# Kyaw-Thiha/animal-vision

Measured on AMD Instinct MI355X. Metric: megapixels/sec per-frame pipeline, higher is better.
Workload: dtype f16

## Files before the change

### animal-vision_amd/csrc/mst_fused.hip

```cpp
#include <hip/hip_fp16.h>

#include <cstdio>
#include <cstdlib>
#include <cstring>

#include "avx_internal.h"
#include "mst_common.h"
#include "mst_tile_order.h"

namespace {

typedef float float4_t __attribute__((ext_vector_type(4)));
#ifndef AVX_FFN32_GM2
#define AVX_FFN32_GM2 1
#endif
constexpr int kFT = 512;
constexpr int TS = 16;
constexpr int HS = TS + 2;
#ifndef AVX_FFN_TH
#define AVX_FFN_TH 16
#endif
constexpr int kFfnTH = AVX_FFN_TH;
static_assert(kFfnTH == 14 || kFfnTH == 16, "FeedForward tile rows");
constexpr int kFfnNGRP = (HS * (kFfnTH + 2) + 31) / 32;

__device__ __forceinline__ float16_t mfma16(half8_t a, half8_t b, float16_t c) { return __builtin_amdgcn_mfma_f32_32x32x16_f16(a, b, c, 0, 0, 0); }

struct Tile { int x0, y0; long b; };
template <class Walk>
__device__ __forceinline__ Tile tile_at(const Walk& wk, int side_x, int side_y) { return Tile{wk.xi * side_x, wk.yi * side_y, (long)wk.b}; }
int mst_tile_order() {
    const char* e = getenv("AVX_MST_TILE_ORDER");
    return e && !strcmp(e, "raster") ? AVX_TILE_ORDER_RASTER : AVX_TILE_ORDER_XCD;
}

typedef _Float16 half16_t __attribute__((ext_vector_type(16)));
template <bool DWS>
__device__ __forceinline__ float4_t dw_unit(const half8_t (&a)[3], const uint4 (&bq)[3]) {
    float4_t acc = {0.f, 0.f, 0.f, 0.f};
    if constexpr (DWS) {
        const half8_t b0 = __builtin_bit_cast(half8_t, bq[0]), b1 = __builtin_bit_cast(half8_t, bq[1]);
        acc = __builtin_amdgcn_mfma_f32_16x16x32_f16(a[1], __builtin_bit_cast(half8_t, bq[2]), acc, 0, 0, 0);
        acc = __builtin_amdgcn_smfmac_f32_16x16x64_f16(a[0], __builtin_shufflevector(b0, b1, 0, 1, 2, 3, 4, 5, 6, 7, 8, 9, 10, 11, 12, 13, 14, 15), acc,
                                                       (int)__builtin_bit_cast(uint4, a[2]).x, 0, 0);
    } else {
#pragma unroll
        for (int i = 0; i < 3; ++i) acc = __builtin_amdgcn_mfma_f32_16x16x32_f16(a[i], __builtin_bit_cast(half8_t, bq[i]), acc, 0, 0, 0);
    }
    return acc;
}
template <bool DWS>
__device__ __forceinline__ half8_t dw_frag(const uint4* p, int i) {
    if (DWS && i == 2) return __builtin_bit_cast(half8_t, uint4{*reinterpret_cast<const unsigned*>(p), 0u, 0u, 0u});
    return __builtin_bit_cast(half8_t, *p);
}
template <bool MARCH> struct FfnWalk { typedef TileWalk type; };
template <> struct FfnWalk<true> { typedef ColumnWalk type; };
template <int C, int HPASS, int MINW, bool DWM, bool STAMP = false, int NW = 8, bool DWS = false, bool MARCH = false>
__global__ __launch_bounds__(64 * NW, MINW) void k_mst_ffn_fused(const __half* __restrict__ x , const float* __restrict__ gamma, const float* __restrict__ beta,
                                                          float eps, const uint4* __restrict__ w1pack , const __half* __restrict__ taps ,
                                                          const uint4* __restrict__ w2pack , __half* __restrict__ out , int B,
                                                          int H, int W, const uint4* __restrict__ dwpack , unsigned long long* __restrict__ stamps , int order ) {
    constexpr int FTH = MARCH ? 14 : kFfnTH, HSY = FTH + 2, ROW0 = MARCH ? 2 : 0, NHALO = HS * (HSY - ROW0), NGRP = (NHALO + 31) / 32;
    constexpr int HID = 4 * C, NPASS = HID / HPASS, KS1 = C / 16, KS2 = HPASS / 16, NT = C / 32, YPITCH = C * 2 + 16, LNV = C / 16;
    constexpr int HPITCH = HPASS * 2 + 16, RPITCH = (HS * HPITCH + 255) / 256 * 256 , NCT = HPASS / 32;
    static_assert(C == 32 || C == 64 || C == 128, "31-, 62- or 124-channel blocks (stored 32 / 64 / 128 wide)");
    constexpr int NTHR = 64 * NW, NGW = (NGRP + NW - 1) / NW;
    constexpr int NTW = NT / (NW / 8), NOCTW = HPASS / (8 * NW);
    static_assert((NW == 8 || NW == 16) && NT % (NW / 8) == 0 && (!DWM || HPASS % (8 * NW) == 0) && (DWM || NW == 8) && (DWM || !DWS) && (DWM || !MARCH), "wave split");
    constexpr bool PREFETCH = C <= 64;
    extern __shared__ __align__(16) unsigned char smem[];
    unsigned char* yt = smem;
    unsigned char* ht = yt + (size_t)NGRP * 32 * YPITCH;
    __half* tapl = reinterpret_cast<__half*>(ht + (size_t)HSY * RPITCH);
    float* gl = reinterpret_cast<float*>(tapl + (DWM ? 0 : 9 * HID));
    constexpr bool W2LDS = NW == 16;
    uint4* w2l = reinterpret_cast<uint4*>(gl + 2 * C);
    constexpr int NPRIME = 2 * HS, CARRY = NPRIME * HPITCH;
    unsigned char* carry = reinterpret_cast<unsigned char*>(w2l + (W2LDS ? NT * KS2 * 64 : 0));
    const int tid = threadIdx.x, lane = tid & 63, wave = tid >> 6, p = lane & 31, h = lane >> 5;
    unsigned long long seg[8] = {0, 0, 0, 0, 0, 0, 0, 0}, tlast = 0;
    auto stamp = [&](int k) {
        if constexpr (STAMP) {
            const unsigned long long now = __builtin_readcyclecounter();
            seg[k] += now - tlast;
            tlast = now;
        }
    };
    if constexpr (STAMP) tlast = __builtin_readcyclecounter();
    if constexpr (!DWM)
        for (int i = tid; i < 9 * HID; i += NTHR) tapl[i] = taps[i];
    for (int i = tid; i < C; i += NTHR) { gl[i] = gamma[i]; gl[C + i] = beta[i]; }
    const int tx = (W + TS - 1) / TS, ty = (H + FTH - 1) / FTH;
    const float cnt = (float)(NT * 31);

    uint4 raw[NGW][LNV];
    unsigned f_rel[NGW];
#pragma unroll
    for (int gi = 0; gi < NGW; ++gi) {
        const int q = 32 * (wave + NW * gi) + p, qq = q < NHALO ? q : NHALO - 1;
        f_rel[gi] = (unsigned)(((qq / HS) * W + qq % HS) * C + h * (C / 2)) * 2u;
    }
    auto fetch = [&](const Tile& t) {
        if (t.y0 + ROW0 >= 1 && t.y0 + HSY - 1 <= H && t.x0 >= 1 && t.x0 + HS - 1 <= W) {
            const char* origin = reinterpret_cast<const char*>(x + ((t.b * H + t.y0 - 1 + ROW0) * (size_t)W + t.x0 - 1) * C);
#pragma unroll
            for (int gi = 0; gi < NGW; ++gi) {
                if (wave + NW * gi >= NGRP) break;
                unsigned o = f_rel[gi];
                asm volatile("" : "+v"(o));
                const uint4* src = reinterpret_cast<const uint4*>(origin + o);
#pragma unroll
                for (int v = 0; v < LNV; ++v) raw[gi][v] = src[v];
            }
            return;
        }
#pragma unroll
        for (int gi = 0; gi < NGW; ++gi) {
            const int g = wave + NW * gi;
            if (g >= NGRP) break;
            const int q = 32 * g + p, qq = q < NHALO ? q : NHALO - 1;
            int yy = t.y0 - 1 + ROW0 + qq / HS, xx = t.x0 - 1 + qq % HS;
            yy = yy < 0 ? 0 : (yy >= H ? H - 1 : yy);
            xx = xx < 0 ? 0 : (xx >= W ? W - 1 : xx);
            const uint4* src = reinterpret_cast<const uint4*>(x + ((t.b * H + yy) * (size_t)W + xx) * C + h * (C / 2));
#pragma unroll
            for (int v = 0; v < LNV; ++v) raw[gi][v] = src[v];
        }
    };
    constexpr int NGPRIME = (NPRIME + 31) / 32;
    auto fetch_prime = [&](const Tile& t) {
        if (wave >= NGPRIME) return;
        int td = tid;
        asm volatile("" : "+v"(td));
        const int q = 32 * (td >> 6) + (td & 31), qq = q < NPRIME ? q : NPRIME - 1, hl = (td >> 5) & 1;
        int yy = t.y0 - 1 + qq / HS, xx = t.x0 - 1 + qq % HS;
        yy = yy < 0 ? 0 : (yy >= H ? H - 1 : yy);
        xx = xx < 0 ? 0 : (xx >= W ? W - 1 : xx);
        const uint4* src = reinterpret_cast<const uint4*>(x + ((t.b * H + yy) * (size_t)W + xx) * C + hl * (C / 2));
#pragma unroll
        for (int v = 0; v < LNV; ++v) raw[0][v] = src[v];
    };
    auto layernorm = [&](int ngrp) {
        if constexpr (DWM) {
#pragma unroll
            for (int gi = 0; gi < NGW; ++gi) {
                const int g = wave + NW * gi;
                if (g >= ngrp) break;
                typedef _Float16 half2v __attribute__((ext_vector_type(2)));
                constexpr unsigned kOnes = 0x3c003c00u;
                auto is_pad = [&](int i) { return ((h * (C / 2) + i) & 31) == 31; };
                auto word = [&](int i) { const uint4 u = raw[gi][i / 8]; const int k = (i / 2) & 3; return k == 0 ? u.x : k == 1 ? u.y : k == 2 ? u.z : u.w; };
                float s1 = 0.f;
#pragma unroll
                for (int i = 0; i < 8 * LNV; i += 2) s1 = __builtin_amdgcn_fdot2(__builtin_bit_cast(half2v, word(i)), __builtin_bit_cast(half2v, kOnes), s1, false);
                const float mean = (s1 + __shfl_xor(s1, 32)) / cnt, nmean = -mean;
                float d[8 * LNV], s2 = 0.f;
#pragma unroll
                for (int i = 0; i < 8 * LNV; ++i) {
                    const float t = (i & 1) ? fma_mix_hi_c(word(i), kOnes, nmean) : fma_mix_lo_c(word(i), kOnes, nmean);
                    d[i] = is_pad(i) ? 0.f : t;
                    s2 = __builtin_fmaf(d[i], d[i], s2);
                }
                const float rstd = rsqrtf((s2 + __shfl_xor(s2, 32)) / cnt + eps);
                int pl = p;
                if constexpr (MARCH) asm volatile("" : "+v"(pl));
                unsigned char* dst = yt + (size_t)(32 * g + pl) * YPITCH + h * C;
#pragma unroll
                for (int v = 0; v < LNV; ++v) {
                    unsigned o[4];
#pragma unroll
                    for (int j = 0; j < 8; j += 2) {
                        const int i = 8 * v + j;
                        const float2_t y2 = float2_t{d[i], d[i + 1]} * float2_t{rstd, rstd};
                        const float bq = (h * (C / 2) + i + 1) == 31 ? 1.0f : y2.y;
                        o[j / 2] = pack_f16(y2.x, bq);
                    }
                    *reinterpret_cast<uint4*>(dst + 16 * v) = uint4{o[0], o[1], o[2], o[3]};
                }
            }
            return;
        }
#pragma unroll
        for (int gi = 0; gi < NGW; ++gi) {
            const int g = wave + NW * gi;
            if (g >= NGRP) break;
            constexpr unsigned kOnes = 0x3c003c00u;
            auto is_pad = [&](int i) { return ((h * (C / 2) + i) & 31) == 31; };
            auto word = [&](int i) { const uint4 u = raw[gi][i / 8]; const int k = (i / 2) & 3; return k == 0 ? u.x : k == 1 ? u.y : k == 2 ? u.z : u.w; };
            float s1 = 0.f;
#pragma unroll
            for (int i = 0; i < 8 * LNV; ++i) {
                const float t = (i & 1) ? fma_mix_hi_c(word(i), kOnes, s1) : fma_mix_lo_c(word(i), kOnes, s1);
                s1 = is_pad(i) ? s1 : t;
            }
            const float mean = (s1 + __shfl_xor(s1, 32)) / cnt, nmean = -mean;
            float d[8 * LNV], s2 = 0.f;
#pragma unroll
            for (int i = 0; i < 8 * LNV; ++i) {
                const float t = (i & 1) ? fma_mix_hi_c(word(i), kOnes, nmean) : fma_mix_lo_c(word(i), kOnes, nmean);
                d[i] = is_pad(i) ? 0.f : t;
                s2 = __builtin_fmaf(d[i], d[i], s2);
            }
            const float rstd = rsqrtf((s2 + __shfl_xor(s2, 32)) / cnt + eps);
            unsigned char* dst = yt + (size_t)(32 * g + p) * YPITCH + h * C;
#pragma unroll
            for (int v = 0; v < LNV; ++v) {
                unsigned o[4];
#pragma unroll
                for (int j = 0; j < 8; j += 2) {
                    const int i = 8 * v + j, c = h * (C / 2) + i;
                    const float a = is_pad(i) ? 0.f : __builtin_fmaf(d[i] * rstd, gl[c], gl[C + c]);
                    const float bq = is_pad(i + 1) ? 0.f : __builtin_fmaf(d[i + 1] * rstd, gl[c + 1], gl[C + c + 1]);
                    o[j / 2] = pack_f16(a, bq);
                }
                *reinterpret_cast<uint4*>(dst + 16 * v) = uint4{o[0], o[1], o[2], o[3]};
            }
        }
    };

    const int n0 = (wave / 8) * NTW, w8 = wave % 8;
    half8_t w2f[W2LDS ? 1 : NTW * KS2];
    auto load_w2 = [&](int pass) {
#pragma unroll
        for (int n = 0; n < NTW; ++n)
#pragma unroll
            for (int s = 0; s < KS2; ++s) w2f[n * KS2 + s] = __builtin_bit_cast(half8_t, w2pack[((size_t)(n0 + n) * (HID / 16) + pass * KS2 + s) * 64 + lane]);
    };
    if constexpr (NPASS == 1 && !W2LDS) load_w2(0);
    half8_t w1f[KS1];
    auto load_w1 = [&](int pass) {
#pragma unroll
        for (int s = 0; s < KS1; ++s) w1f[s] = __builtin_bit_cast(half8_t, w1pack[((size_t)(pass * NCT + wave % NCT) * KS1 + s) * 64 + lane]);
    };
    constexpr bool W1AHEAD = DWM && C == 64 && NPASS > 1 && NW == 8;
    static_assert(!(MARCH && W1AHEAD), "the marching form loads W1 at the top of phase 1 (priming replaces the fragments)");
    if constexpr (W1AHEAD) load_w1(0);
    constexpr int NITEM = (NGRP + NW / NCT - 1) / (NW / NCT);
    int p1_g[NITEM], p1_dst[NITEM], p1_dy[NITEM], p1_dx[NITEM];
#pragma unroll
    for (int j = 0; j < NITEM; ++j) {
        const int g = wave / NCT + j * (NW / NCT), q = 32 * g + p, qc = q < NHALO ? q : 0;
        p1_g[j] = g < NGRP ? g : -1;
        p1_dst[j] = (g < NGRP && q < NHALO) ? (ROW0 + qc / HS) * RPITCH + (qc % HS) * HPITCH + 32 * h : -1;
        p1_dy[j] = ROW0 + qc / HS - 1; p1_dx[j] = qc % HS - 1;
    }
    auto p1_item = [&](int g, unsigned char* base, int off, bool masked, int yy, int xx) {
        float16_t d;
#pragma unroll
        for (int v = 0; v < 16; ++v) d[v] = 0.f;
        const unsigned char* ysrc = yt + (size_t)(32 * g + p) * YPITCH + 16 * h;
#pragma unroll
        for (int s = 0; s < KS1; ++s) d = mfma16(w1f[s], __builtin_bit_cast(half8_t, *reinterpret_cast<const uint4*>(ysrc + 32 * s)), d);
        if (off >= 0) {
            unsigned char* dst = base + off;
            uint32_t keep = 0xffffffffu;
            if (masked) keep = (yy >= 0 && yy < H && xx >= 0 && xx < W) ? 0xffffffffu : 0u;
            constexpr int GP1 = (C == 64 && NW == 8) ? 4 : (C == 32 ? 2 : 1);
            unsigned pk[8];
#pragma unroll
            for (int v0 = 0; v0 < 8; v0 += GP1) {
                float2_t gq[GP1];
#pragma unroll
                for (int v = 0; v < GP1; ++v) gq[v] = float2_t{d[2 * (v0 + v)], d[2 * (v0 + v) + 1]};
                if constexpr (DWM) gelu_mx<GP1>(gq); else gelu_multi<GP1>(gq);
#pragma unroll
                for (int v = 0; v < GP1; ++v) pk[v0 + v] = pack_f16(gq[v].x, gq[v].y);
            }
            uint4 u0 = uint4{pk[0], pk[1], pk[2], pk[3]}, u1 = uint4{pk[4], pk[5], pk[6], pk[7]};
            if (masked) { u0.x &= keep; u0.y &= keep; u0.z &= keep; u0.w &= keep; u1.x &= keep; u1.y &= keep; u1.z &= keep; u1.w &= keep; }
            reinterpret_cast<uint4*>(dst)[0] = u0;
            reinterpret_cast<uint4*>(dst)[1] = u1;
        }
    };
    auto prime = [&](const Tile& t) {
        fetch_prime(t);
        layernorm(NGPRIME);
        __syncthreads();
        const int g = wave / NCT;
        int td = tid;
        asm volatile("" : "+v"(td));
        const int wl = td >> 6, q = 32 * (wl / NCT) + (td & 31), qc = q < NPRIME ? q : 0, yy = t.y0 - 1 + qc / HS, xx = t.x0 - 1 + qc % HS;
        const int off = q < NPRIME ? qc * HPITCH + 32 * ((td >> 5) & 1) + 64 * (wl % NCT) : -1;
        if (g < NGPRIME) {
#pragma unroll 1
            for (int pass = 0; pass < NPASS; ++pass) {
                load_w1(pass);
                p1_item(g, carry + (size_t)pass * CARRY, off, true, yy, xx);
            }
        }
        __syncthreads();
    };
    typename FfnWalk<MARCH>::type ahead;
    if constexpr (MARCH) ahead.init(blockIdx.x, gridDim.x, B, ty, tx);
    else ahead.init(blockIdx.x, gridDim.x, B, ty, tx, order);
    if (!ahead.live) return;
    Tile t = tile_at(ahead, TS, FTH);
    ahead.advance();
    if constexpr (MARCH) prime(t);
    fetch(t);
    __syncthreads();
    layernorm(NGRP);
    for (;;) {
        const bool halo_inside = t.y0 + ROW0 >= 1 && t.y0 + HSY - 1 <= H && t.x0 >= 1 && t.x0 + HS - 1 <= W;
        float16_t D[NTW];
#pragma unroll
        for (int n = 0; n < NTW; ++n)
#pragma unroll
            for (int v = 0; v < 16; ++v) D[n][v] = 0.f;
#pragma unroll 1
        for (int pass = 0; pass < NPASS; ++pass) {
            stamp(pass == 0 ? 7 : 5);
            __syncthreads();
            stamp(0);
            if constexpr (W2LDS)
                for (int i = tid; i < NT * KS2 * 64; i += NTHR) w2l[i] = w2pack[((size_t)(i / (KS2 * 64)) * (HID / 16) + pass * KS2 + (i / 64) % KS2) * 64 + (i & 63)];
            half8_t af[DWM ? NOCTW : 1][3];
            if constexpr (DWM) {
#pragma unroll
                for (int o2 = 0; o2 < NOCTW; ++o2)
#pragma unroll
                    for (int i = 0; i < 3; ++i) af[o2][i] = dw_frag<DWS>(dwpack + ((size_t)(pass * (HPASS / 8) + NW * o2 + wave) * 3 + i) * 64 + lane, i);
            }
            {
                const int ct = wave % NCT;
                if constexpr (!W1AHEAD) load_w1(pass);
                if constexpr (MARCH) {
                    constexpr int NV = NPRIME * (HPASS / 8);
                    static_assert(NV <= NTHR, "one 16-byte piece per thread");
                    int i = tid;
                    asm volatile("" : "+v"(i));
                    if (i < NV) {
                        const int px = i / (HPASS / 8), o = i % (HPASS / 8);
                        *reinterpret_cast<uint4*>(ht + (size_t)(px / HS) * RPITCH + (size_t)(px % HS) * HPITCH + 16 * o) =
                            *reinterpret_cast<const uint4*>(carry + (size_t)pass * CARRY + (size_t)px * HPITCH + 16 * o);
                    }
                }
#pragma unroll
                for (int j = 0; j < NITEM; ++j) {
                    if (p1_g[j] < 0) continue;
                    p1_item(p1_g[j], ht + 64 * ct, p1_dst[j], !halo_inside, t.y0 + p1_dy[j], t.x0 + p1_dx[j]);
                }
            }
            stamp(1);
            __syncthreads();
            stamp(2);
            bool ahead_fetch = ahead.live;
            if constexpr (MARCH) ahead_fetch = ahead_fetch && !ahead.seg;
            if (PREFETCH && pass == NPASS - 1 && ahead_fetch) fetch(tile_at(ahead, TS, FTH));
            if constexpr (NPASS > 1 && !W2LDS) load_w2(pass);
            if constexpr (DWM) {
                constexpr int NOCT = NOCTW;
                const int n16 = lane & 15, q = lane >> 4;
                unsigned char* rbase = ht + (size_t)q * RPITCH + (size_t)n16 * HPITCH + 16 * wave;
                unsigned char* wbase = ht + (size_t)(q >> 1) * RPITCH + (size_t)n16 * HPITCH + 16 * wave + 8 * (q & 1);
                constexpr int NU = NOCT * (FTH / 2);
                uint4 bq[3];
                auto rd = [&](int u) {
                    const int o2 = u / (FTH / 2), pr = u % (FTH / 2);
#pragma unroll
                    for (int i = 0; i < 3; ++i) bq[i] = *reinterpret_cast<const uint4*>(rbase + (size_t)(2 * pr) * RPITCH + (size_t)i * HPITCH + 16 * NW * o2);
                };
                auto finish = [&](int u, float4_t a) {
                    const int o2 = u / (FTH / 2), pr = u % (FTH / 2);
                    float2_t gp[2] = {float2_t{a[0], a[1]}, float2_t{a[2], a[3]}};
                    if constexpr (C == 64 || (C == 32 && AVX_FFN32_GM2)) gelu_mx<2>(gp);
                    else { float2_t g0[1] = {gp[0]}, g1[1] = {gp[1]}; gelu_mx<1>(g0); gelu_mx<1>(g1); gp[0] = g0[0]; gp[1] = g1[0]; }
                    *reinterpret_cast<uint2*>(wbase + (size_t)(2 * pr) * RPITCH + 16 * NW * o2) = uint2{pack_f16(gp[0].x, gp[0].y), pack_f16(gp[1].x, gp[1].y)};
                };
#ifndef AVX_FFN_PIPE_ALL
#define AVX_FFN_PIPE_ALL 0
#endif
#ifndef AVX_FFN_MARCH_PIPE32
#define AVX_FFN_MARCH_PIPE32 1
#endif
                constexpr bool PIPE = C == 64 || AVX_FFN_PIPE_ALL || (MARCH && C == 32 && AVX_FFN_MARCH_PIPE32);
                if constexpr (PIPE) {
                    rd(0);
                    float4_t prev = {0.f, 0.f, 0.f, 0.f};
#pragma unroll
                    for (int u = 0; u < NU; ++u) {
                        const int o2 = u / (FTH / 2);
                        const float4_t acc = dw_unit<DWS>(af[o2], bq);
                        if (u + 1 < NU) rd(u + 1);
                        __builtin_amdgcn_sched_barrier(0);
                        if (u > 0) finish(u - 1, prev);
                        __builtin_amdgcn_sched_barrier(0);
                        prev = acc;
                    }
                    finish(NU - 1, prev);
                } else {
#pragma unroll
                    for (int u = 0; u < NU; ++u) {
                        const int o2 = u / (FTH / 2);
                        rd(u);
                        const float4_t acc = dw_unit<DWS>(af[o2], bq);
                        finish(u, acc);
                    }
                }
                stamp(3);
                __syncthreads();
                stamp(4);
                if constexpr (W1AHEAD) load_w1(pass + 1 < NPASS ? pass + 1 : 0);
                const int r = 2 * w8 + (p >> 4), c = p & 15;
                const unsigned char* zb = ht + (size_t)r * RPITCH + (size_t)c * HPITCH + 16 * h;
                constexpr int NVC = NPRIME * (HPASS / 8);
                constexpr bool SPREAD = MARCH && !W2LDS;
                uint4 cv = uint4{0u, 0u, 0u, 0u};
                int ci = tid;
                if constexpr (SPREAD) {
                    asm volatile("" : "+v"(ci));
                    if (ci < NVC) cv = *reinterpret_cast<const uint4*>(ht + (size_t)(FTH + (ci / (HPASS / 8)) / HS) * RPITCH + (size_t)((ci / (HPASS / 8)) % HS) * HPITCH + 16 * (ci % (HPASS / 8)));
                }
                if (SPREAD || 2 * w8 < FTH) {
#pragma unroll
                for (int s = 0; s < KS2; ++s) {
                    const half8_t bf = __builtin_bit_cast(half8_t, *reinterpret_cast<const uint4*>(zb + 32 * s));
#pragma unroll
                    for (int n = 0; n < NTW; ++n) {
                        if constexpr (W2LDS) D[n] = mfma16(__builtin_bit_cast(half8_t, w2l[((n0 + n) * KS2 + s) * 64 + lane]), bf, D[n]);
                        else D[n] = mfma16(w2f[n * KS2 + s], bf, D[n]);
                    }
                }
                }
                if constexpr (SPREAD) {
                    if (ci < NVC) *reinterpret_cast<uint4*>(carry + (size_t)pass * CARRY + (size_t)(ci / (HPASS / 8)) * HPITCH + 16 * (ci % (HPASS / 8))) = cv;
                } else if constexpr (MARCH) {
                    if (2 * w8 >= FTH)
                        for (int i = (wave / 8) * 64 + lane; i < NVC; i += 64 * (NW / 8)) {
                            const int px = i / (HPASS / 8), o = i % (HPASS / 8);
                            *reinterpret_cast<uint4*>(carry + (size_t)pass * CARRY + (size_t)px * HPITCH + 16 * o) =
                                *reinterpret_cast<const uint4*>(ht + (size_t)(FTH + px / HS) * RPITCH + (size_t)(px % HS) * HPITCH + 16 * o);
                        }
                }
            } else
            if (2 * wave < FTH) {
                const int r = 2 * wave + (p >> 4), c = p & 15;
                const unsigned char* hbase = ht + (size_t)r * RPITCH + (size_t)c * HPITCH + 16 * h;
                const unsigned char* tbase = reinterpret_cast<const unsigned char*>(tapl) + (size_t)(pass * HPASS + 8 * h) * 2;
#pragma unroll
                for (int s = 0; s < KS2; ++s) {
                    float acc[8];
#pragma unroll
                    for (int j = 0; j < 8; ++j) acc[j] = 0.f;
#pragma unroll
                    for (int tap = 0; tap < 9; ++tap) {
                        const uint4 hv = *reinterpret_cast<const uint4*>(hbase + (size_t)(tap / 3) * RPITCH + (size_t)(tap % 3) * HPITCH + 32 * s);
                        const uint4 wv = *reinterpret_cast<const uint4*>(tbase + (size_t)tap * HID * 2 + 32 * s);
                        fma_mix_lo(acc[0], hv.x, wv.x); fma_mix_hi(acc[1], hv.x, wv.x);
                        fma_mix_lo(acc[2], hv.y, wv.y); fma_mix_hi(acc[3], hv.y, wv.y);
                        fma_mix_lo(acc[4], hv.z, wv.z); fma_mix_hi(acc[5], hv.z, wv.z);
                        fma_mix_lo(acc[6], hv.w, wv.w); fma_mix_hi(acc[7], hv.w, wv.w);
                    }
                    half8_t bf;
#pragma unroll
                    for (int j = 0; j < 8; j += 2) {
                        const float2_t gv = gelu_fast2(float2_t{acc[j], acc[j + 1]});
                        bf[j] = (_Float16)gv.x;
                        bf[j + 1] = (_Float16)gv.y;
                    }
#pragma unroll
                    for (int n = 0; n < NT; ++n)
                        D[n] = mfma16(w2f[n * KS2 + s], bf, D[n]);
                }
            }
        }
        stamp(5);
        {
            const int yo = t.y0 + 2 * w8 + (p >> 4), xo = t.x0 + (p & 15);
            if (2 * w8 < FTH && yo < H && xo < W) {
                const size_t off = ((t.b * H + yo) * (size_t)W + xo) * C + 16 * h + 32 * n0;
#pragma unroll
                for (int n = 0; n < NTW; ++n) {
                    const uint4 xa = reinterpret_cast<const uint4*>(x + off + 32 * n)[0], xb = reinterpret_cast<const uint4*>(x + off + 32 * n)[1];
                    const unsigned xw[8] = {xa.x, xa.y, xa.z, xa.w, xb.x, xb.y, xb.z, xb.w};
                    unsigned ow[8];
#pragma unroll
                    for (int j = 0; j < 8; ++j) {
                        float s0 = D[n][2 * j], s1 = D[n][2 * j + 1];
                        fma_mix_lo(s0, xw[j], 0x3c003c00u); fma_mix_hi(s1, xw[j], 0x3c003c00u);
                        ow[j] = pack_f16(s0, s1);
                    }
                    reinterpret_cast<uint4*>(out + off + 32 * n)[0] = uint4{ow[0], ow[1], ow[2], ow[3]};
                    reinterpret_cast<uint4*>(out + off + 32 * n)[1] = uint4{ow[4], ow[5], ow[6], ow[7]};
                }
            }
        }
        stamp(6);
        if (!ahead.live) break;
        t = tile_at(ahead, TS, FTH);
        bool fetch_now = !PREFETCH;
        if constexpr (MARCH) {
            if (ahead.seg) { prime(t); fetch_now = true; }
        }
        ahead.advance();
        if (fetch_now) fetch(t);
        layernorm(NGRP);
    }
    if constexpr (STAMP) {
        if (lane == 0 && stamps)
#pragma unroll
            for (int k = 0; k < 8; ++k) stamps[((size_t)blockIdx.x * NW + wave) * 8 + k] = seg[k];
    }
}


constexpr int VS = TS + 4, MS = TS + 2;

template <int C, int MINW>
__global__ __launch_bounds__(kFT, MINW) void k_mst_attn_tail(const __half* __restrict__ v , const __half* __restrict__ x ,
                                                             const uint4* __restrict__ mpack , const __half* __restrict__ taps1 ,
                                                             const __half* __restrict__ taps2 , const float* __restrict__ bias ,
                                                             __half* __restrict__ out, int B, int H, int W, const uint4* __restrict__ wvpack ) {
    constexpr int NO = C / 8, NS = C / 16, NT = C / 32, PP = C * 2 + 16;
    constexpr int VRP = (VS * PP + 255) / 256 * 256, MRP = VRP;
    constexpr int NFILL = (VS * VS * NO + kFT - 1) / kFT;
    extern __shared__ __align__(16) unsigned char smem[];
    unsigned char* vt = smem;
    unsigned char* mt = vt + (size_t)VS * VRP;
    const bool fromx = wvpack != nullptr;
    __half* t2l = reinterpret_cast<__half*>(mt + (size_t)VS * VRP);
    __half* t1l = t2l + 9 * C;
    float* bl = reinterpret_cast<float*>(t1l + 9 * C);
    const int tid = threadIdx.x, lane = tid & 63, wave = tid >> 6, p = lane & 31, h = lane >> 5;
// ... 1387 lines not shown
}

extern "C" int avx_mst_ffn_fused(avx_ctx* ctx, const void* x, const float* gamma, const float* beta, float eps, const void* w1pack, const void* taps_9xhid,
                                 const void* w2pack, void* out, int B, int H, int W, int C, void* stream) {
    if (!ctx) return AVX_ERR_INVALID;
    AVX_REQUIRE(ctx, taps_9xhid, "avx_mst_ffn_fused: NULL pointer");
    return ffn_fused_launch(ctx, x, gamma, beta, eps, w1pack, taps_9xhid, nullptr, w2pack, out, B, H, W, C, stream);
}

extern "C" int avx_mst_ffn_fused_mx(avx_ctx* ctx, const void* x, const float* gamma, const float* beta, float eps, const void* w1pack, const void* dwpack,
                                    const void* w2pack, void* out, int B, int H, int W, int C, void* stream) {
    if (!ctx) return AVX_ERR_INVALID;
    AVX_REQUIRE(ctx, dwpack && (((uintptr_t)dwpack) & 15u) == 0, "avx_mst_ffn_fused_mx: dwpack NULL or not 16-byte aligned");
    return ffn_fused_launch(ctx, x, gamma, beta, eps, w1pack, nullptr, dwpack, w2pack, out, B, H, W, C, stream);
}

extern "C" int avx_mst_ffn_fused_sp(avx_ctx* ctx, const void* x, const float* gamma, const float* beta, float eps, const void* w1pack, const void* dwpack,
                                    const void* w2pack, void* out, int B, int H, int W, int C, void* stream) {
    if (!ctx) return AVX_ERR_INVALID;
    AVX_REQUIRE(ctx, dwpack && (((uintptr_t)dwpack) & 15u) == 0, "avx_mst_ffn_fused_sp: dwpack NULL or not 16-byte aligned");
    return ffn_fused_launch(ctx, x, gamma, beta, eps, w1pack, nullptr, dwpack, w2pack, out, B, H, W, C, stream, true);
}

extern "C" int avx_mst_ffn_fused_mx_col(avx_ctx* ctx, const void* x, const float* gamma, const float* beta, float eps, const void* w1pack, const void* dwpack,
                                        const void* w2pack, void* out, int B, int H, int W, int C, int max_workgroups, void* stream) {
    if (!ctx) return AVX_ERR_INVALID;
    AVX_REQUIRE(ctx, dwpack && (((uintptr_t)dwpack) & 15u) == 0, "avx_mst_ffn_fused_mx_col: dwpack NULL or not 16-byte aligned");
    AVX_REQUIRE(ctx, (C == 32 || C == 64) && max_workgroups >= 0, "avx_mst_ffn_fused_mx_col: C=%d (32 or 64), max_workgroups=%d (>= 0)", C, max_workgroups);
    return ffn_fused_launch(ctx, x, gamma, beta, eps, w1pack, nullptr, dwpack, w2pack, out, B, H, W, C, stream, false, true, max_workgroups);
}
extern "C" int avx_mst_ffn_fused_sp_col(avx_ctx* ctx, const void* x, const float* gamma, const float* beta, float eps, const void* w1pack, const void* dwpack,
                                        const void* w2pack, void* out, int B, int H, int W, int C, int max_workgroups, void* stream) {
    if (!ctx) return AVX_ERR_INVALID;
    AVX_REQUIRE(ctx, dwpack && (((uintptr_t)dwpack) & 15u) == 0, "avx_mst_ffn_fused_sp_col: dwpack NULL or not 16-byte aligned");
    AVX_REQUIRE(ctx, (C == 32 || C == 64) && max_workgroups >= 0, "avx_mst_ffn_fused_sp_col: C=%d (32 or 64), max_workgroups=%d (>= 0)", C, max_workgroups);
    return ffn_fused_launch(ctx, x, gamma, beta, eps, w1pack, nullptr, dwpack, w2pack, out, B, H, W, C, stream, true, true, max_workgroups);
}

static int ffn_fused_launch(avx_ctx* ctx, const void* x, const float* gamma, const float* beta, float eps, const void* w1pack, const void* taps_9xhid, const void* dwpack,
                            const void* w2pack, void* out, int B, int H, int W, int C, void* stream, bool sparse, bool march, int max_workgroups) {
    AVX_REQUIRE(ctx, x && gamma && beta && w1pack && w2pack && out && B > 0 && H > 0 && W > 0, "avx_mst_ffn_fused: NULL pointer or empty tensor");
    AVX_REQUIRE(ctx, C == 32 || C == 64 || C == 128, "avx_mst_ffn_fused: C=%d (32, 64 or 128: 31-channel groups stored 32 wide)", C);
    AVX_REQUIRE(ctx, ((((uintptr_t)x | (uintptr_t)w1pack | (uintptr_t)w2pack | (uintptr_t)out | (uintptr_t)taps_9xhid)) & 15u) == 0,
                "avx_mst_ffn_fused: pointers must be 16-byte aligned");
    AVX_REQUIRE(ctx, x != out, "avx_mst_ffn_fused: neighbouring tiles read each other's halo: the output cannot be the input");
    AVX_HIP(ctx, hipSetDevice(ctx->device));
    hipStream_t s = avx_pick_stream(ctx, stream);
    const int fth = march ? 14 : kFfnTH;
    const long total = (long)B * ((H + fth - 1) / fth) * ((W + TS - 1) / TS);
    const char* hp = getenv("AVX_MST_FFN_HPASS");
    const bool small = C == 32 && (march || !(hp && atoi(hp) == 128));
    const int hpass = (small || C == 128) ? 64 : 128, hpitch = hpass * 2 + 16, rpitch = (HS * hpitch + 255) / 256 * 256;
    const long cap = (long)ctx->num_cus * (small ? 2 : 1);
    const bool nw16 = C == 64 && dwpack && (march || !(getenv("AVX_MST_FFN_NW") && atoi(getenv("AVX_MST_FFN_NW")) == 8));
    const size_t lds = (size_t)(march ? 8 : kFfnNGRP) * 32 * (C * 2 + 16) + (size_t)(fth + 2) * rpitch + (dwpack ? 0 : (size_t)9 * 4 * C * 2) + sizeof(float) * 2 * C +
                       (nw16 ? (size_t)(C / 32) * (hpass / 16) * 1024 : 0) + (march ? (size_t)(4 * C / hpass) * 2 * HS * hpitch : 0);
    AVX_REQUIRE(ctx, total <= 0x7fffffffl, "avx_mst_ffn_fused: 2^31 tiles or more");
    AVX_REQUIRE(ctx, !march || (dwpack && (C == 32 || C == 64)), "avx_mst_ffn_fused: the marching form is built for the matrix-pipe kernels at C = 32 and 64");
    long nwg = total < cap ? total : cap;
    if (max_workgroups > 0 && max_workgroups < nwg) nwg = max_workgroups;
    const dim3 grid((unsigned)nwg);
    const int order = mst_tile_order();
#define AVX_FFN1M(CV, HP, MW, DW, NWV, SP, MR)                                                                                                   \
    {                                                                                                                                            \
        auto k = k_mst_ffn_fused<CV, HP, MW, DW, false, NWV, SP, MR>;                                                                            \
        AVX_HIP(ctx, hipFuncSetAttribute((const void*)k, hipFuncAttributeMaxDynamicSharedMemorySize, (int)lds));                                 \
        hipLaunchKernelGGL(k, grid, dim3(64 * NWV), lds, s, (const __half*)x, gamma, beta, eps, (const uint4*)w1pack, (const __half*)taps_9xhid, \
                           (const uint4*)w2pack, (__half*)out, B, H, W, (const uint4*)dwpack, (unsigned long long*)nullptr, order);              \
    }
#define AVX_FFN1S(CV, HP, MW, DW, NWV, SP) AVX_FFN1M(CV, HP, MW, DW, NWV, SP, false)
#define AVX_FFN1(CV, HP, MW, DW, NWV) AVX_FFN1S(CV, HP, MW, DW, NWV, false)
#define AVX_FFN(CV, HP, MW) { if (dwpack && sparse) AVX_FFN1S(CV, HP, MW, true, 8, true) else if (dwpack) AVX_FFN1(CV, HP, MW, true, 8) else AVX_FFN1(CV, HP, MW, false, 8) }
    if (dwpack && getenv("AVX_FFN_STAMPS") && ((C == 32 && small) || C == 64 || C == 128)) {
        unsigned long long* d_st = nullptr;
        const int nwv = nw16 ? 16 : 8;
        const size_t n = (size_t)grid.x * nwv * 8;
        AVX_HIP(ctx, hipMalloc((void**)&d_st, n * sizeof(unsigned long long)));
#define AVX_FFN_ST2(CV, HP, MW, NWV, SP, MR)                                                                                                     \
    {                                                                                                                                            \
        auto k = k_mst_ffn_fused<CV, HP, MW, true, true, NWV, SP, MR>;                                                                           \
        AVX_HIP(ctx, hipFuncSetAttribute((const void*)k, hipFuncAttributeMaxDynamicSharedMemorySize, (int)lds));                                 \
        hipLaunchKernelGGL(k, grid, dim3(64 * NWV), lds, s, (const __half*)x, gamma, beta, eps, (const uint4*)w1pack, (const __half*)taps_9xhid, \
                           (const uint4*)w2pack, (__half*)out, B, H, W, (const uint4*)dwpack, d_st, order);                                      \
    }
#define AVX_FFN_ST1(CV, HP, MW, NWV, SP) AVX_FFN_ST2(CV, HP, MW, NWV, SP, false)
#define AVX_FFN_ST(CV, HP, MW, NWV) { if (sparse) AVX_FFN_ST1(CV, HP, MW, NWV, true) else AVX_FFN_ST1(CV, HP, MW, NWV, false) }
#define AVX_FFN_STM(CV, HP, MW, NWV) { if (sparse) AVX_FFN_ST2(CV, HP, MW, NWV, true, true) else AVX_FFN_ST2(CV, HP, MW, NWV, false, true) }
        if (march && C == 32) AVX_FFN_STM(32, 64, 4, 8) else if (march) AVX_FFN_STM(64, 128, 1, 16)
        else if (C == 32) AVX_FFN_ST(32, 64, 4, 8) else if (nw16) AVX_FFN_ST(64, 128, 1, 16) else if (C == 64) AVX_FFN_ST(64, 128, 2, 8) else AVX_FFN_ST(128, 64, 2, 8)
#undef AVX_FFN_STM
#undef AVX_FFN_ST
#undef AVX_FFN_ST1
#undef AVX_FFN_ST2
        AVX_HIP(ctx, hipStreamSynchronize(s));
        unsigned long long* h_st = (unsigned long long*)malloc(n * sizeof(unsigned long long));
        AVX_HIP(ctx, hipMemcpy(h_st, d_st, n * sizeof(unsigned long long), hipMemcpyDeviceToHost));
        double tot[8] = {0}, w0[8] = {0}, w7[8] = {0};
        for (size_t i = 0; i < n; ++i) { tot[i & 7] += (double)h_st[i]; if (((i >> 3) % nwv) == 0) w0[i & 7] += (double)h_st[i]; if (((i >> 3) % nwv) == (size_t)nwv - 1) w7[i & 7] += (double)h_st[i]; }
        double all = 0;
        for (int k2 = 0; k2 < 8; ++k2) all += tot[k2];
        fprintf(stderr, "[ffn stamps C=%d%s] %u blocks x %d waves, mean cycles per wave %.0f; share per segment (all waves | first wave | last wave): ", C, march ? " march" : "", grid.x, nwv, all / (grid.x * (double)nwv));
        const char* nm[8] = {"bar1", "phase1", "bar2", "phase2a", "bar3", "phase2b", "epilogue", "ln+fetch"};
        for (int k2 = 0; k2 < 8; ++k2) fprintf(stderr, "%s %.1f%% | %.1f%% | %.1f%%  ", nm[k2], 100 * tot[k2] / all, 100 * w0[k2] * nwv / all, 100 * w7[k2] * nwv / all);
        fprintf(stderr, "\n");
        free(h_st);
        (void)hipFree(d_st);
    } else if (march && C == 32 && sparse) AVX_FFN1M(32, 64, 4, true, 8, true, true)
    else if (march && C == 32) AVX_FFN1M(32, 64, 4, true, 8, false, true)
    else if (march && sparse) AVX_FFN1M(64, 128, 1, true, 16, true, true)
    else if (march) AVX_FFN1M(64, 128, 1, true, 16, false, true)
    else if (C == 32 && small) AVX_FFN(32, 64, 4) else if (C == 32) AVX_FFN(32, 128, 2)
    else if (nw16 && sparse) AVX_FFN1S(64, 128, 1, true, 16, true)
    else if (nw16) AVX_FFN1(64, 128, 1, true, 16)
    else if (C == 64) AVX_FFN(64, 128, 2) else AVX_FFN(128, 64, 2)
#undef AVX_FFN
#undef AVX_FFN1
#undef AVX_FFN1S
#undef AVX_FFN1M
    AVX_HIP(ctx, hipGetLastError());
    return AVX_OK;
}

extern "C" int avx_mst_attn_tail(avx_ctx* ctx, const void* v, const void* x, const void* mpack16, const void* taps1_9xc, const void* taps2_9xc, const float* bias,
                                 void* out, int B, int H, int W, int C, void* stream) {
    if (!ctx) return AVX_ERR_INVALID;
    AVX_REQUIRE(ctx, v && x && mpack16 && taps1_9xc && taps2_9xc && out && B > 0 && H > 0 && W > 0, "avx_mst_attn_tail: NULL pointer or empty tensor");
    AVX_REQUIRE(ctx, C == 32 || C == 64, "avx_mst_attn_tail: C=%d (32 or 64)", C);
    AVX_REQUIRE(ctx, ((((uintptr_t)v | (uintptr_t)x | (uintptr_t)mpack16 | (uintptr_t)out | (uintptr_t)taps1_9xc | (uintptr_t)taps2_9xc)) & 15u) == 0,
                "avx_mst_attn_tail: pointers must be 16-byte aligned");
    AVX_REQUIRE(ctx, v != out, "avx_mst_attn_tail: tiles read their neighbours' rows of v: the output cannot be v (it may be x)");
    AVX_HIP(ctx, hipSetDevice(ctx->device));
    hipStream_t s = avx_pick_stream(ctx, stream);
    if (C == 32) return launch_attn_tail<32, 4>(ctx, v, x, mpack16, taps1_9xc, taps2_9xc, bias, out, B, H, W, s, nullptr);
    return launch_attn_tail<64, 2>(ctx, v, x, mpack16, taps1_9xc, taps2_9xc, bias, out, B, H, W, s, nullptr);
}

extern "C" int avx_mst_attn_tail_x(avx_ctx* ctx, const void* x, const void* wvpack16, const void* mpack16, const void* taps1_9xc, const void* taps2_9xc,
                                   const float* bias, void* out, int B, int H, int W, int C, void* stream) {
    if (!ctx) return AVX_ERR_INVALID;
    AVX_REQUIRE(ctx, x && wvpack16 && mpack16 && taps1_9xc && taps2_9xc && out && B > 0 && H > 0 && W > 0, "avx_mst_attn_tail_x: NULL pointer or empty tensor");
    AVX_REQUIRE(ctx, C == 32 || C == 64, "avx_mst_attn_tail_x: C=%d (32 or 64)", C);
    AVX_REQUIRE(ctx, ((((uintptr_t)x | (uintptr_t)wvpack16 | (uintptr_t)mpack16 | (uintptr_t)out | (uintptr_t)taps1_9xc | (uintptr_t)taps2_9xc)) & 15u) == 0,
                "avx_mst_attn_tail_x: pointers must be 16-byte aligned");
    AVX_REQUIRE(ctx, x != out, "avx_mst_attn_tail_x: tiles read their neighbours' rows of x: the output cannot be x");
    AVX_HIP(ctx, hipSetDevice(ctx->device));
    hipStream_t s = avx_pick_stream(ctx, stream);
    if (C == 32) return launch_attn_tail<32, 4>(ctx, x, x, mpack16, taps1_9xc, taps2_9xc, bias, out, B, H, W, s, wvpack16);
    return launch_attn_tail<64, 2>(ctx, x, x, mpack16, taps1_9xc, taps2_9xc, bias, out, B, H, W, s, wvpack16);
}

template <bool DWS>
static int attn_tail_mx_launch(avx_ctx* ctx, const void* x, const void* wvpack16, const void* mpack_mx, const void* dw1pack, const void* dw2pack, const float* bias, void* out,
                               int B, int H, int W, int C, void* stream) {
    AVX_REQUIRE(ctx, x && wvpack16 && mpack_mx && dw1pack && dw2pack && out && B > 0 && H > 0 && W > 0, "avx_mst_attn_tail_mx: NULL pointer or empty tensor");
    AVX_REQUIRE(ctx, C == 32 || C == 64 || C == 128, "avx_mst_attn_tail_mx: C=%d (32, 64 or 128)", C);
    AVX_REQUIRE(ctx, ((((uintptr_t)x | (uintptr_t)wvpack16 | (uintptr_t)mpack_mx | (uintptr_t)out | (uintptr_t)dw1pack | (uintptr_t)dw2pack)) & 15u) == 0,
                "avx_mst_attn_tail_mx: pointers must be 16-byte aligned");
    AVX_REQUIRE(ctx, x != out, "avx_mst_attn_tail_mx: tiles read their neighbours' rows of x: the output cannot be x");
    AVX_HIP(ctx, hipSetDevice(ctx->device));
    hipStream_t s = avx_pick_stream(ctx, stream);
    if (C == 32) return launch_attn_tail_mx<32, 16, 4, 8, DWS>(ctx, x, wvpack16, mpack_mx, dw1pack, dw2pack, bias, out, B, H, W, s);
    if (C == 128) return launch_attn_tail_mx<128, 8, 2, 8, DWS>(ctx, x, wvpack16, mpack_mx, dw1pack, dw2pack, bias, out, B, H, W, s);
    if (getenv("AVX_MST_TAIL_NW") && atoi(getenv("AVX_MST_TAIL_NW")) == 16) return launch_attn_tail_mx<64, 16, 1, 16, DWS>(ctx, x, wvpack16, mpack_mx, dw1pack, dw2pack, bias, out, B, H, W, s);
    return launch_attn_tail_mx<64, 16, 2, 8, DWS>(ctx, x, wvpack16, mpack_mx, dw1pack, dw2pack, bias, out, B, H, W, s);
// ... 256 lines not shown
```

Baseline: 456.5.

## Run C=128 FeedForward with 16 waves, splitting depthwise row pairs across two waves

```diff
diff --git a/animal-vision_amd/csrc/mst_fused.hip b/animal-vision_amd/csrc/mst_fused.hip
--- a/animal-vision_amd/csrc/mst_fused.hip
+++ b/animal-vision_amd/csrc/mst_fused.hip
@@ -3,6 +3,7 @@
 #include <cstdio>
 #include <cstdlib>
 #include <cstring>
+#include <type_traits>
 
 #include "avx_internal.h"
 #include "mst_common.h"
@@ -66,16 +67,31 @@
     constexpr int HPITCH = HPASS * 2 + 16, RPITCH = (HS * HPITCH + 255) / 256 * 256 , NCT = HPASS / 32;
     static_assert(C == 32 || C == 64 || C == 128, "31-, 62- or 124-channel blocks (stored 32 / 64 / 128 wide)");
     constexpr int NTHR = 64 * NW, NGW = (NGRP + NW - 1) / NW;
-    constexpr int NTW = NT / (NW / 8), NOCTW = HPASS / (8 * NW);
-    static_assert((NW == 8 || NW == 16) && NT % (NW / 8) == 0 && (!DWM || HPASS % (8 * NW) == 0) && (DWM || NW == 8) && (DWM || !DWS) && (DWM || !MARCH), "wave split");
-    constexpr bool PREFETCH = C <= 64;
+    constexpr bool SPLIT = DWM && 2 * HPASS == 8 * NW;
+    constexpr int NTW = NT / (NW / 8), NOCTW = SPLIT ? 1 : HPASS / (8 * NW);
+    static_assert((NW == 8 || NW == 16) && NT % (NW / 8) == 0 && (!DWM || SPLIT || HPASS % (8 * NW) == 0) && (DWM || NW == 8) && (DWM || !DWS) && (DWM || !MARCH), "wave split");
+    static_assert(!SPLIT || (!MARCH && FTH == 16 && NW == 16), "two waves per octet: 8 row pairs, 4 each");
+#ifndef AVX_FFN128_PREFETCH
+#define AVX_FFN128_PREFETCH 0
+#endif
+#ifndef AVX_FFN128_PIPE
+#define AVX_FFN128_PIPE 1
+#endif
+#ifndef AVX_FFN128_GP1
+#define AVX_FFN128_GP1 1
+#endif
+#ifndef AVX_FFN128_W1AHEAD
+#define AVX_FFN128_W1AHEAD 1
+#endif
+    constexpr bool PREFETCH = C <= 64 || (SPLIT && AVX_FFN128_PREFETCH);
+    constexpr int YTPX = SPLIT ? NHALO : NGRP * 32;
     extern __shared__ __align__(16) unsigned char smem[];
     unsigned char* yt = smem;
-    unsigned char* ht = yt + (size_t)NGRP * 32 * YPITCH;
+    unsigned char* ht = yt + (size_t)YTPX * YPITCH;
     __half* tapl = reinterpret_cast<__half*>(ht + (size_t)HSY * RPITCH);
     float* gl = reinterpret_cast<float*>(tapl + (DWM ? 0 : 9 * HID));
     constexpr bool W2LDS = NW == 16;
-    uint4* w2l = reinterpret_cast<uint4*>(gl + 2 * C);
+    uint4* w2l = reinterpret_cast<uint4*>(gl + (SPLIT ? 0 : 2 * C));
     constexpr int NPRIME = 2 * HS, CARRY = NPRIME * HPITCH;
     unsigned char* carry = reinterpret_cast<unsigned char*>(w2l + (W2LDS ? NT * KS2 * 64 : 0));
     const int tid = threadIdx.x, lane = tid & 63, wave = tid >> 6, p = lane & 31, h = lane >> 5;
@@ -90,7 +106,8 @@
     if constexpr (STAMP) tlast = __builtin_readcyclecounter();
     if constexpr (!DWM)
         for (int i = tid; i < 9 * HID; i += NTHR) tapl[i] = taps[i];
-    for (int i = tid; i < C; i += NTHR) { gl[i] = gamma[i]; gl[C + i] = beta[i]; }
+    if constexpr (!SPLIT)
+        for (int i = tid; i < C; i += NTHR) { gl[i] = gamma[i]; gl[C + i] = beta[i]; }
     const int tx = (W + TS - 1) / TS, ty = (H + FTH - 1) / FTH;
     const float cnt = (float)(NT * 31);
 
@@ -106,7 +123,7 @@
             const char* origin = reinterpret_cast<const char*>(x + ((t.b * H + t.y0 - 1 + ROW0) * (size_t)W + t.x0 - 1) * C);
 #pragma unroll
             for (int gi = 0; gi < NGW; ++gi) {
-                if (wave + NW * gi >= NGRP) break;
+                if (!SPLIT && wave + NW * gi >= NGRP) break;
                 unsigned o = f_rel[gi];
                 asm volatile("" : "+v"(o));
                 const uint4* src = reinterpret_cast<const uint4*>(origin + o);
@@ -118,12 +135,15 @@
 #pragma unroll
         for (int gi = 0; gi < NGW; ++gi) {
             const int g = wave + NW * gi;
-            if (g >= NGRP) break;
-            const int q = 32 * g + p, qq = q < NHALO ? q : NHALO - 1;
+            if (!SPLIT && g >= NGRP) break;
+            int tb = tid;
+            if constexpr (SPLIT) asm volatile("" : "+v"(tb));
+            const int pb = SPLIT ? tb & 31 : p, hb = SPLIT ? (tb >> 5) & 1 : h;
+            const int q = 32 * g + pb, qq = q < NHALO ? q : NHALO - 1;
             int yy = t.y0 - 1 + ROW0 + qq / HS, xx = t.x0 - 1 + qq % HS;
             yy = yy < 0 ? 0 : (yy >= H ? H - 1 : yy);
             xx = xx < 0 ? 0 : (xx >= W ? W - 1 : xx);
-            const uint4* src = reinterpret_cast<const uint4*>(x + ((t.b * H + yy) * (size_t)W + xx) * C + h * (C / 2));
+            const uint4* src = reinterpret_cast<const uint4*>(x + ((t.b * H + yy) * (size_t)W + xx) * C + hb * (C / 2));
 #pragma unroll
             for (int v = 0; v < LNV; ++v) raw[gi][v] = src[v];
         }
@@ -155,12 +175,17 @@
 #pragma unroll
                 for (int i = 0; i < 8 * LNV; i += 2) s1 = __builtin_amdgcn_fdot2(__builtin_bit_cast(half2v, word(i)), __builtin_bit_cast(half2v, kOnes), s1, false);
                 const float mean = (s1 + __shfl_xor(s1, 32)) / cnt, nmean = -mean;
-                float d[8 * LNV], s2 = 0.f;
+                float d[SPLIT ? 1 : 8 * LNV], s2 = 0.f, nmean2 = nmean;
+                if constexpr (SPLIT) asm volatile("" : "+v"(nmean2));
+                auto centred = [&](int i, float nm) {
+                    const float t = (i & 1) ? fma_mix_hi_c(word(i), kOnes, nm) : fma_mix_lo_c(word(i), kOnes, nm);
+                    return is_pad(i) ? 0.f : t;
+                };
 #pragma unroll
                 for (int i = 0; i < 8 * LNV; ++i) {
-                    const float t = (i & 1) ? fma_mix_hi_c(word(i), kOnes, nmean) : fma_mix_lo_c(word(i), kOnes, nmean);
-                    d[i] = is_pad(i) ? 0.f : t;
-                    s2 = __builtin_fmaf(d[i], d[i], s2);
+                    const float di = centred(i, nmean);
+                    if constexpr (!SPLIT) d[i] = di;
+                    s2 = __builtin_fmaf(di, di, s2);
                 }
                 const float rstd = rsqrtf((s2 + __shfl_xor(s2, 32)) / cnt + eps);
                 int pl = p;
@@ -172,11 +197,14 @@
 #pragma unroll
                     for (int j = 0; j < 8; j += 2) {
                         const int i = 8 * v + j;
-                        const float2_t y2 = float2_t{d[i], d[i + 1]} * float2_t{rstd, rstd};
+                        float2_t dd;
+                        if constexpr (SPLIT) dd = float2_t{centred(i, nmean2), centred(i + 1, nmean2)};
+                        else dd = float2_t{d[i], d[i + 1]};
+                        const float2_t y2 = dd * float2_t{rstd, rstd};
                         const float bq = (h * (C / 2) + i + 1) == 31 ? 1.0f : y2.y;
                         o[j / 2] = pack_f16(y2.x, bq);
                     }
-                    *reinterpret_cast<uint4*>(dst + 16 * v) = uint4{o[0], o[1], o[2], o[3]};
+                    if (YTPX == NGRP * 32 || 32 * g + pl < YTPX) *reinterpret_cast<uint4*>(dst + 16 * v) = uint4{o[0], o[1], o[2], o[3]};
                 }
             }
             return;
@@ -233,7 +261,7 @@
 #pragma unroll
         for (int s = 0; s < KS1; ++s) w1f[s] = __builtin_bit_cast(half8_t, w1pack[((size_t)(pass * NCT + wave % NCT) * KS1 + s) * 64 + lane]);
     };
-    constexpr bool W1AHEAD = DWM && C == 64 && NPASS > 1 && NW == 8;
+    constexpr bool W1AHEAD = DWM && NPASS > 1 && ((C == 64 && NW == 8) || (SPLIT && AVX_FFN128_W1AHEAD));
     static_assert(!(MARCH && W1AHEAD), "the marching form loads W1 at the top of phase 1 (priming replaces the fragments)");
     if constexpr (W1AHEAD) load_w1(0);
     constexpr int NITEM = (NGRP + NW / NCT - 1) / (NW / NCT);
@@ -249,14 +277,15 @@
         float16_t d;
 #pragma unroll
         for (int v = 0; v < 16; ++v) d[v] = 0.f;
-        const unsigned char* ysrc = yt + (size_t)(32 * g + p) * YPITCH + 16 * h;
+        const int ypx = (YTPX == NGRP * 32 || 32 * g + p < YTPX) ? 32 * g + p : YTPX - 1;
+        const unsigned char* ysrc = yt + (size_t)ypx * YPITCH + 16 * h;
 #pragma unroll
         for (int s = 0; s < KS1; ++s) d = mfma16(w1f[s], __builtin_bit_cast(half8_t, *reinterpret_cast<const uint4*>(ysrc + 32 * s)), d);
         if (off >= 0) {
             unsigned char* dst = base + off;
             uint32_t keep = 0xffffffffu;
             if (masked) keep = (yy >= 0 && yy < H && xx >= 0 && xx < W) ? 0xffffffffu : 0u;
-            constexpr int GP1 = (C == 64 && NW == 8) ? 4 : (C == 32 ? 2 : 1);
+            constexpr int GP1 = (C == 64 && NW == 8) ? 4 : (C == 32 ? 2 : (SPLIT ? AVX_FFN128_GP1 : 1));
             unsigned pk[8];
 #pragma unroll
             for (int v0 = 0; v0 < 8; v0 += GP1) {
@@ -320,7 +349,7 @@
 #pragma unroll
                 for (int o2 = 0; o2 < NOCTW; ++o2)
 #pragma unroll
-                    for (int i = 0; i < 3; ++i) af[o2][i] = dw_frag<DWS>(dwpack + ((size_t)(pass * (HPASS / 8) + NW * o2 + wave) * 3 + i) * 64 + lane, i);
+                    for (int i = 0; i < 3; ++i) af[o2][i] = dw_frag<DWS>(dwpack + ((size_t)(pass * (HPASS / 8) + (SPLIT ? wave % 8 : NW * o2 + wave)) * 3 + i) * 64 + lane, i);
             }
             {
                 const int ct = wave % NCT;
@@ -352,21 +381,25 @@
             if constexpr (DWM) {
                 constexpr int NOCT = NOCTW;
                 const int n16 = lane & 15, q = lane >> 4;
-                unsigned char* rbase = ht + (size_t)q * RPITCH + (size_t)n16 * HPITCH + 16 * wave;
-                unsigned char* wbase = ht + (size_t)(q >> 1) * RPITCH + (size_t)n16 * HPITCH + 16 * wave + 8 * (q & 1);
-                constexpr int NU = NOCT * (FTH / 2);
+                const int ow = SPLIT ? wave % 8 : wave;
+                unsigned char* rbase = ht + (size_t)q * RPITCH + (size_t)n16 * HPITCH + 16 * ow;
+                unsigned char* wbase = ht + (size_t)(q >> 1) * RPITCH + (size_t)n16 * HPITCH + 16 * ow + 8 * (q & 1);
+                constexpr int NPR = SPLIT ? FTH / 4 : FTH / 2;
+                constexpr int NU = NOCT * NPR;
+                auto run2a = [&](auto hfc) {
+                constexpr bool HF = decltype(hfc)::value;
                 uint4 bq[3];
                 auto rd = [&](int u) {
-                    const int o2 = u / (FTH / 2), pr = u % (FTH / 2);
+                    const int o2 = u / NPR, pr = HF ? FTH / 2 - 1 - u % NPR : u % NPR;
 #pragma unroll
                     for (int i = 0; i < 3; ++i) bq[i] = *reinterpret_cast<const uint4*>(rbase + (size_t)(2 * pr) * RPITCH + (size_t)i * HPITCH + 16 * NW * o2);
                 };
                 auto finish = [&](int u, float4_t a) {
-                    const int o2 = u / (FTH / 2), pr = u % (FTH / 2);
+                    const int o2 = u / NPR, pr = HF ? FTH / 2 - 1 - u % NPR : u % NPR;
                     float2_t gp[2] = {float2_t{a[0], a[1]}, float2_t{a[2], a[3]}};
                     if constexpr (C == 64 || (C == 32 && AVX_FFN32_GM2)) gelu_mx<2>(gp);
                     else { float2_t g0[1] = {gp[0]}, g1[1] = {gp[1]}; gelu_mx<1>(g0); gelu_mx<1>(g1); gp[0] = g0[0]; gp[1] = g1[0]; }
-                    *reinterpret_cast<uint2*>(wbase + (size_t)(2 * pr) * RPITCH + 16 * NW * o2) = uint2{pack_f16(gp[0].x, gp[0].y), pack_f16(gp[1].x, gp[1].y)};
+                    *reinterpret_cast<uint2*>(wbase + (size_t)(2 * pr + (HF ? 2 : 0)) * RPITCH + 16 * NW * o2) = uint2{pack_f16(gp[0].x, gp[0].y), pack_f16(gp[1].x, gp[1].y)};
                 };
 #ifndef AVX_FFN_PIPE_ALL
 #define AVX_FFN_PIPE_ALL 0
@@ -374,13 +407,13 @@
 #ifndef AVX_FFN_MARCH_PIPE32
 #define AVX_FFN_MARCH_PIPE32 1
 #endif
-                constexpr bool PIPE = C == 64 || AVX_FFN_PIPE_ALL || (MARCH && C == 32 && AVX_FFN_MARCH_PIPE32);
+                constexpr bool PIPE = C == 64 || AVX_FFN_PIPE_ALL || (MARCH && C == 32 && AVX_FFN_MARCH_PIPE32) || (SPLIT && AVX_FFN128_PIPE);
                 if constexpr (PIPE) {
                     rd(0);
                     float4_t prev = {0.f, 0.f, 0.f, 0.f};
 #pragma unroll
                     for (int u = 0; u < NU; ++u) {
-                        const int o2 = u / (FTH / 2);
+                        const int o2 = u / NPR;
                         const float4_t acc = dw_unit<DWS>(af[o2], bq);
                         if (u + 1 < NU) rd(u + 1);
                         __builtin_amdgcn_sched_barrier(0);
@@ -392,17 +425,21 @@
                 } else {
 #pragma unroll
                     for (int u = 0; u < NU; ++u) {
-                        const int o2 = u / (FTH / 2);
+                        const int o2 = u / NPR;
                         rd(u);
                         const float4_t acc = dw_unit<DWS>(af[o2], bq);
                         finish(u, acc);
                     }
                 }
+                };
+                if constexpr (SPLIT) {
+                    if (__builtin_amdgcn_readfirstlane(wave) >= 8) run2a(std::true_type{}); else run2a(std::false_type{});
+                } else run2a(std::false_type{});
                 stamp(3);
                 __syncthreads();
                 stamp(4);
                 if constexpr (W1AHEAD) load_w1(pass + 1 < NPASS ? pass + 1 : 0);
-                const int r = 2 * w8 + (p >> 4), c = p & 15;
+                const int r = 2 * w8 + (p >> 4) + (SPLIT && w8 >= 4 ? 2 : 0), c = p & 15;
                 const unsigned char* zb = ht + (size_t)r * RPITCH + (size_t)c * HPITCH + 16 * h;
                 constexpr int NVC = NPRIME * (HPASS / 8);
                 constexpr bool SPREAD = MARCH && !W2LDS;
@@ -467,9 +504,12 @@
         }
         stamp(5);
         {
-            const int yo = t.y0 + 2 * w8 + (p >> 4), xo = t.x0 + (p & 15);
+            int te = tid;
+            if constexpr (SPLIT) asm volatile("" : "+v"(te));
+            const int pe = SPLIT ? te & 31 : p, he = SPLIT ? (te >> 5) & 1 : h;
+            const int yo = t.y0 + 2 * w8 + (pe >> 4), xo = t.x0 + (pe & 15);
             if (2 * w8 < FTH && yo < H && xo < W) {
-                const size_t off = ((t.b * H + yo) * (size_t)W + xo) * C + 16 * h + 32 * n0;
+                const size_t off = ((t.b * H + yo) * (size_t)W + xo) * C + 16 * he + 32 * n0;
 #pragma unroll
                 for (int n = 0; n < NTW; ++n) {
                     const uint4 xa = reinterpret_cast<const uint4*>(x + off + 32 * n)[0], xb = reinterpret_cast<const uint4*>(x + off + 32 * n)[1];
@@ -1963,11 +2003,13 @@
     const bool small = C == 32 && (march || !(hp && atoi(hp) == 128));
     const int hpass = (small || C == 128) ? 64 : 128, hpitch = hpass * 2 + 16, rpitch = (HS * hpitch + 255) / 256 * 256;
     const long cap = (long)ctx->num_cus * (small ? 2 : 1);
-    const bool nw16 = C == 64 && dwpack && (march || !(getenv("AVX_MST_FFN_NW") && atoi(getenv("AVX_MST_FFN_NW")) == 8));
-    const size_t lds = (size_t)(march ? 8 : kFfnNGRP) * 32 * (C * 2 + 16) + (size_t)(fth + 2) * rpitch + (dwpack ? 0 : (size_t)9 * 4 * C * 2) + sizeof(float) * 2 * C +
-                       (nw16 ? (size_t)(C / 32) * (hpass / 16) * 1024 : 0) + (march ? (size_t)(4 * C / hpass) * 2 * HS * hpitch : 0);
+    const bool nw16 = (C == 64 || C == 128) && dwpack && (march || !(getenv("AVX_MST_FFN_NW") && atoi(getenv("AVX_MST_FFN_NW")) == 8));
+    const bool split = nw16 && C == 128;
+    const size_t lds = (split ? (size_t)HS * (fth + 2) : (size_t)(march ? 8 : kFfnNGRP) * 32) * (C * 2 + 16) + (size_t)(fth + 2) * rpitch + (dwpack ? 0 : (size_t)9 * 4 * C * 2) +
+                       (split ? 0 : sizeof(float) * 2 * C) + (nw16 ? (size_t)(C / 32) * (hpass / 16) * 1024 : 0) + (march ? (size_t)(4 * C / hpass) * 2 * HS * hpitch : 0);
     AVX_REQUIRE(ctx, total <= 0x7fffffffl, "avx_mst_ffn_fused: 2^31 tiles or more");
     AVX_REQUIRE(ctx, !march || (dwpack && (C == 32 || C == 64)), "avx_mst_ffn_fused: the marching form is built for the matrix-pipe kernels at C = 32 and 64");
+    AVX_REQUIRE(ctx, lds <= 163840, "avx_mst_ffn_fused: %zu bytes of LDS, a CU has 163,840", lds);
     long nwg = total < cap ? total : cap;
     if (max_workgroups > 0 && max_workgroups < nwg) nwg = max_workgroups;
     const dim3 grid((unsigned)nwg);
@@ -1998,7 +2040,7 @@
 #define AVX_FFN_ST(CV, HP, MW, NWV) { if (sparse) AVX_FFN_ST1(CV, HP, MW, NWV, true) else AVX_FFN_ST1(CV, HP, MW, NWV, false) }
 #define AVX_FFN_STM(CV, HP, MW, NWV) { if (sparse) AVX_FFN_ST2(CV, HP, MW, NWV, true, true) else AVX_FFN_ST2(CV, HP, MW, NWV, false, true) }
         if (march && C == 32) AVX_FFN_STM(32, 64, 4, 8) else if (march) AVX_FFN_STM(64, 128, 1, 16)
-        else if (C == 32) AVX_FFN_ST(32, 64, 4, 8) else if (nw16) AVX_FFN_ST(64, 128, 1, 16) else if (C == 64) AVX_FFN_ST(64, 128, 2, 8) else AVX_FFN_ST(128, 64, 2, 8)
+        else if (C == 32) AVX_FFN_ST(32, 64, 4, 8) else if (split) AVX_FFN_ST(128, 64, 1, 16) else if (nw16) AVX_FFN_ST(64, 128, 1, 16) else if (C == 64) AVX_FFN_ST(64, 128, 2, 8) else AVX_FFN_ST(128, 64, 2, 8)
 #undef AVX_FFN_STM
 #undef AVX_FFN_ST
 #undef AVX_FFN_ST1
@@ -2021,6 +2063,8 @@
     else if (march && sparse) AVX_FFN1M(64, 128, 1, true, 16, true, true)
     else if (march) AVX_FFN1M(64, 128, 1, true, 16, false, true)
     else if (C == 32 && small) AVX_FFN(32, 64, 4) else if (C == 32) AVX_FFN(32, 128, 2)
+    else if (split && sparse) AVX_FFN1S(128, 64, 1, true, 16, true)
+    else if (split) AVX_FFN1(128, 64, 1, true, 16)
     else if (nw16 && sparse) AVX_FFN1S(64, 128, 1, true, 16, true)
     else if (nw16) AVX_FFN1(64, 128, 1, true, 16)
     else if (C == 64) AVX_FFN(64, 128, 2) else AVX_FFN(128, 64, 2)
```

Result: no change. 458.3 (median of 6 runs) (+0.4%).
